# pyannote/pyannote-video

Measured on AMD Instinct MI355X. Metric: frames/sec end-to-end detect->embed->cluster, 1080p@25fps, higher is better.
Workload: dtype f32 (detector scores, embedder) / f64 (tracker, clustering) / u8 frames; an f16 screening pass with a proven error bound decides which windows the detector's exact f32 chain is evaluated for -- results identical to dense f32 scoring (`dense_scoring`)

## Files before the change

include/pvface.h:

```cpp
#ifndef PVFACE_H
#define PVFACE_H
#include <stdint.h>
#include <stddef.h>

#ifdef __cplusplus
extern "C" {
#endif

typedef uint64_t pvf_handle;
typedef struct { int32_t left, top, right, bottom; } pvf_rect_i32;

const char* pvf_last_error(void);
int32_t pvf_version(void);
int32_t pvf_device_count(int32_t* n);
int32_t pvf_ctx_create(int32_t device, pvf_handle* ctx);
int32_t pvf_ctx_create_prio(int32_t device, int32_t priority_class, pvf_handle* ctx);
int32_t pvf_ctx_destroy(pvf_handle ctx);
int32_t pvf_sync(pvf_handle ctx);

int32_t pvf_load_detector(pvf_handle ctx, const char* path);
int32_t pvf_load_shape_predictor(pvf_handle ctx, const char* path);
int32_t pvf_load_embedder(pvf_handle ctx, const char* path);
int32_t pvf_model_tensor(const char* path, int32_t kind, const char* name, void* out, int64_t cap_bytes, int64_t* nbytes);
int32_t pvf_set_tracker_tables(pvf_handle ctx, const double* mask64, const double* mask_scale, const double* tw64,
// ... 49 lines not shown
int32_t pvf_egress_create(pvf_handle ctx, int32_t out_w, int32_t out_h, int32_t depth, int32_t flags, pvf_handle* ring);
int32_t pvf_egress_destroy(pvf_handle ctx, pvf_handle ring);
int32_t pvf_egress_submit(pvf_handle ctx, pvf_handle ring, pvf_handle frame, const pvf_prim* prims, int32_t n_prims,
                          const uint8_t* text, int64_t text_bytes, int32_t* slot);
int32_t pvf_egress_wait(pvf_handle ctx, pvf_handle ring, int32_t slot, const uint8_t** host_planes);
int32_t pvf_egress_release(pvf_handle ctx, pvf_handle ring, int32_t slot);
int32_t pvf_debug_render_rgb(pvf_handle ctx, pvf_handle frame, int32_t out_w, int32_t out_h, const pvf_prim* prims, int32_t n_prims,
                             const uint8_t* text, int64_t text_bytes, uint8_t* rgb);
int32_t pvf_debug_redact_means(pvf_handle ctx, pvf_handle frame, int32_t out_w, int32_t out_h, const pvf_prim* prims, int32_t n_prims,
                               uint8_t* means, int64_t capacity);

int32_t pvf_detect(pvf_handle ctx, pvf_handle frame, int32_t upsample, double adjust_threshold,
                   pvf_rect_i32* out, float* scores, int32_t cap, int32_t* n);
int32_t pvf_detect_batch(pvf_handle ctx, const pvf_handle* frames, int32_t n_frames, int32_t upsample,
                         double adjust_threshold, pvf_rect_i32* out, float* scores, int32_t* counts,
                         int32_t cap_per_frame);
int32_t pvf_detect_many(pvf_handle ctx, const pvf_handle* frames, int32_t n_frames, int32_t batch, int32_t upsample,
                        double adjust_threshold, pvf_rect_i32* out, float* scores, int32_t* counts, int32_t cap);

int32_t pvf_detector_screening(pvf_handle ctx, int32_t on, int32_t list_cap);
int32_t pvf_detector_screening_stats(pvf_handle ctx, int64_t* batches, int64_t* listed, int64_t* retries, double* bounds, double* pipe_err);

int32_t pvf_embedder_split(pvf_handle ctx, int32_t on);
int32_t pvf_embedder_split_stats(pvf_handle ctx, int64_t* faces, int64_t* reruns, double* pipe_err);

int32_t pvf_tracker_create(pvf_handle ctx, pvf_handle* trk);
int32_t pvf_tracker_create_many(pvf_handle ctx, int32_t n, pvf_handle* trks);
int32_t pvf_tracker_destroy_many(pvf_handle ctx, const pvf_handle* trks, int32_t n);
int32_t pvf_tracker_clone_many(pvf_handle ctx, const pvf_handle* src, int32_t n, pvf_handle* dst);
int32_t pvf_tracker_destroy(pvf_handle ctx, pvf_handle trk);
int32_t pvf_tracker_start(pvf_handle ctx, pvf_handle trk, pvf_handle frame, const double box[4]);
int32_t pvf_tracker_update(pvf_handle ctx, pvf_handle trk, pvf_handle frame, double* psr);
int32_t pvf_tracker_position(pvf_handle ctx, pvf_handle trk, double box[4]);
int32_t pvf_tracker_start_many(pvf_handle ctx, const pvf_handle* trks, const pvf_handle* frames,
                               const double* boxes , int32_t n);
int32_t pvf_tracker_update_many(pvf_handle ctx, const pvf_handle* trks, const pvf_handle* frames, int32_t n,
                                double* psr , double* boxes_out );
int32_t pvf_tracker_update_many_deferred(pvf_handle ctx, const pvf_handle* trks, const pvf_handle* frames, int32_t n,
                                         double* psr, double* boxes_out);
int32_t pvf_tracker_commit_many(pvf_handle ctx, const pvf_handle* trks, const pvf_handle* frames, int32_t n);

int32_t pvf_overlap_matrix(const double* a, int32_t na, const double* b, int32_t nb, double ratio, double* out);
int32_t pvf_associate(const double* trackers, int32_t n_trackers, const double* detections, int32_t n_detections,
                      double min_overlap_ratio, int32_t* det_of_tracker);
int32_t pvf_munkres(const double* cost, int32_t n, int32_t* row_to_col);

// ... 219 lines not shown
```

pyannote-video_amd/csrc/api.hip:

```cpp
#include "pvf_internal.h"
#include <algorithm>
#include <cmath>
#include <cstdlib>
#include <string>
#include <thread>

#define API_BEGIN try {
#define API_END                                                        \
    return 0;                                                          \
    }                                                                  \
    catch (const std::exception& e) { pvf_set_error(e.what()); return -1; } \
    catch (...) { pvf_set_error("unknown error"); return -2; }

#define ENTER(c, h)                                                \
    Ctx* c = pvf_ctx(h);                                           \
    std::lock_guard<std::recursive_mutex> _api_lock(c->api_mu);    \
    HIP_CHECK(hipSetDevice(c->device))
#define ENTER_DET(c, h)                                            \
    Ctx* c = pvf_ctx(h);                                           \
    std::lock_guard<std::recursive_mutex> _det_lock(c->det_mu);    \
    HIP_CHECK(hipSetDevice(c->device))
#define ENTER_BOTH(c, h)                                           \
    Ctx* c = pvf_ctx(h);                                           \
    std::lock_guard<std::recursive_mutex> _det_lock(c->det_mu);    \
// ... 29 lines not shown
    PVF_REQUIRE(list_cap >= 0 && list_cap <= (1 << 26), "pvf_detector_screening: list_cap must be 0 (keep) .. 2^26");
    c->det_screen = on != 0;
    if (list_cap > 0) c->screen_list_cap = list_cap;
    API_END
}

extern "C" int32_t pvf_detector_screening_stats(pvf_handle h, int64_t* batches, int64_t* listed, int64_t* retries, double* bounds, double* pipe_err)
{
    API_BEGIN
    ENTER_DET(c, h);
    if (batches) *batches = c->screen_batches;
    if (listed) *listed = c->screen_listed;
    if (retries) *retries = c->screen_retries;
    if (bounds) for (int f = 0; f < c->det.n_filters; ++f) bounds[f] = c->det.screen_bound[f];
    if (pipe_err) *pipe_err = c->screen_pipe_err;
    API_END
}

extern "C" int32_t pvf_embedder_split(pvf_handle h, int32_t on)
{
    API_BEGIN
    ENTER(c, h);
    c->emb_split = on != 0;
    API_END
}

extern "C" int32_t pvf_embedder_split_stats(pvf_handle h, int64_t* faces, int64_t* reruns, double* pipe_err)
{
    API_BEGIN
    ENTER(c, h);
    if (faces) *faces = c->emb_split_faces;
    if (reruns) *reruns = c->emb_reruns;
    if (pipe_err) *pipe_err = c->emb_pipe_err;
    API_END
}

extern "C" int32_t pvf_detect_batch(pvf_handle h, const pvf_handle* frames, int32_t n_frames, int32_t upsample, double adjust,
                                    pvf_rect_i32* out, float* scores, int32_t* counts, int32_t cap)
{
    API_BEGIN
    ENTER_DET(c, h);
    PVF_REQUIRE(n_frames > 0 && frames && out && counts && cap > 0, "pvf_detect_batch: bad arguments");
    PVF_REQUIRE(upsample >= 0 && upsample <= 2, "pvf_detect_batch: upsample must be 0..2");
    std::vector<Frame> fr(n_frames);
    for (int i = 0; i < n_frames; ++i) fr[i] = c->frame(frames[i]);
    std::vector<std::vector<RawDet>> raw;
// ... 1160 lines not shown
```

pyannote-video_amd/csrc/ctx.hip:

```cpp
#include "pvf_internal.h"
#include "detect_ml.h"
#include <cmath>
#include <fstream>
#include <mutex>
#include <dlfcn.h>

static thread_local std::string g_err;
void pvf_set_error(const char* msg) { g_err = msg ? msg : ""; }
extern "C" const char* pvf_last_error(void) { return g_err.c_str(); }

static std::mutex g_ctx_mu;
static std::unordered_map<uint64_t, std::unique_ptr<Ctx>> g_ctxs;
static uint64_t g_next_ctx = 0x1000;

Ctx* pvf_ctx(pvf_handle h)
{
    std::lock_guard<std::mutex> lk(g_ctx_mu);
    auto it = g_ctxs.find(h);
    if (it == g_ctxs.end()) throw PvfError("unknown context handle");
    return it->second.get();
}

std::map<std::string, Tensor> pvf_read_container(const char* path)
{
// ... 264 lines not shown
{
    API_BEGIN
    int k = 0;
    if (hipGetDeviceCount(&k) != hipSuccess || k <= 0) throw PvfError("no HIP device visible: libpvface has no CPU fallback");
    PVF_REQUIRE(device >= 0 && device < k, "device index out of range");
    HIP_CHECK(hipSetDevice(device));
    hipDeviceProp_t prop;
    HIP_CHECK(hipGetDeviceProperties(&prop, device));
    if (strncmp(prop.gcnArchName, "gfx950", 6) != 0)
        throw PvfError(std::string("libpvface is built for gfx950 (MI355X) only; device is ") + prop.gcnArchName);
    std::unique_ptr<Ctx> c(new Ctx());
    c->device = device;
    c->n_cu = prop.multiProcessorCount;
    {
        int lo = 0, hi = 0;
        HIP_CHECK(hipDeviceGetStreamPriorityRange(&lo, &hi));
        int prio = priority_class < 0 ? lo : hi;
        if (const char* e = getenv("PVF_MAIN_STREAM_PRIO")) prio = (strcmp(e, "low") == 0) ? lo : hi;
        HIP_CHECK(hipStreamCreateWithPriority(&c->stream, hipStreamNonBlocking, priority_class == 2 ? lo : prio));
        HIP_CHECK(hipStreamCreateWithPriority(&c->det_stream, hipStreamNonBlocking, priority_class == 2 ? hi : lo));
    }
    if (const char* e = getenv("PVF_DETECTOR_SCREENING")) c->det_screen = atoi(e) != 0;
    if (const char* e = getenv("PVF_EMBEDDER_SPLIT")) c->emb_split = atoi(e) != 0;
    std::lock_guard<std::mutex> lk(g_ctx_mu);
    uint64_t id = g_next_ctx++;
    g_ctxs[id] = std::move(c);
    *out = id;
    API_END
}

extern "C" int32_t pvf_ctx_create(int32_t device, pvf_handle* out) { return pvf_ctx_create_prio(device, 0, out); }

extern "C" int32_t pvf_ctx_destroy(pvf_handle h)
{
    API_BEGIN
    Ctx* c = pvf_ctx(h);
    HIP_CHECK(hipSetDevice(c->device));
    (void)hipStreamSynchronize(c->stream);
    (void)hipStreamSynchronize(c->det_stream);
    for (auto& kv : c->frames) if (kv.second.owned) (void)hipFree((void*)kv.second.d);
    for (auto& kv : c->trackers) {
        Tracker& t = *kv.second;
        if (t.share) { if (--*t.share > 0) continue; delete t.share; t.share = nullptr; }
        if (t.d_state) (void)hipFree(t.d_state);
    }
    for (auto p : c->tracker_pool) (void)hipFree(p);
// ... 251 lines not shown
```

pyannote-video_amd/csrc/pvf_internal.h:

```cpp
#pragma once
#include <hip/hip_runtime.h>
#include <cstdint>
#include <cstdio>
#include <cstring>
#include <deque>
#include <map>
#include <atomic>
#include <memory>
#include <mutex>
#include <stdexcept>
#include <string>
#include <unordered_map>
#include <vector>
#include "../../include/pvface.h"
#include "scratch_layout.h"
#include "chip_plan.h"
#include "group_blocks.h"

#define PVF_FHOG_STRIDE 32

struct CandOverflow : PvfError { int needed; explicit CandOverflow(int n) : PvfError("detector: candidate buffer overflow"), needed(n) {} };
struct ScreenRetry : PvfError { ScreenRetry() : PvfError("detector: screening pass gave up") {} };

#define HIP_CHECK(expr)                                                                              \
// ... 186 lines not shown
    std::recursive_mutex api_mu;
    std::recursive_mutex det_mu;
    std::mutex frames_mu;
    std::mutex prof_mu;
    bool prof_on = false;
    std::map<std::string, ProfFamily> prof;
    std::vector<hipEvent_t> event_pool;
    DevBuf s_grad, s_pyr, s_hist, s_norm, s_feat, s_cand, s_misc, s_chip, s_chip_pyr, s_act0, s_act1, s_act2, s_trk0, s_trk1, s_trk2, s_trkfeat, s_clu0, s_clu1;
    HostBuf h_cand, h_misc;
    StageRing stage;
    DevBuf s_cand2[2], s_fptr[2];
    HostBuf h_cand2[2], h_fptr[2];
    hipEvent_t det_ev[2] = {nullptr, nullptr};
    int det_slot = 0;
    int det_cand_cap = 8192;
    bool det_screen = true, det_screen_suspended = false, screen_attr_set = false;
    int screen_list_cap = 1 << 20;
    DevBuf s_screen;
    int64_t screen_batches = 0, screen_listed = 0, screen_retries = 0;
    double screen_pipe_err = -1;
    bool screen_pipe_flushes_subnormals = false;
    bool emb_split = true, emb_probe_done = false;
    DevBuf s_emb_flags, s_emb_redo;
    DevBuf s_jit;
    bool jit_attr_set = false;
    int64_t emb_split_faces = 0, emb_reruns = 0;
    double emb_pipe_err = -1;
    int n_cu = 256;
    struct PoolBuf { uint8_t* p; hipEvent_t free_after; hipEvent_t free_after_det; };
    std::map<size_t, std::deque<PoolBuf>> frame_pool;
    size_t frame_pool_bytes = 0;
    void* ingest_rings = nullptr;
    void* render_state = nullptr;
    void* tube_state = nullptr;
    void* board_state = nullptr;
    struct MlPlanCache* ml_plans = nullptr;
    std::map<std::vector<int>, std::unique_ptr<DevBuf>> resize_tabs;
    const void* feat_ring_owner = nullptr;
    uint8_t* d_orient_lut = nullptr;
    uint8_t* d_wrap_lut = nullptr;
    DevBuf s_orb_set, s_orb_work;
    int orb_n = 0, orb_cap = 0;

    Frame frame(uint64_t id)
    {
        std::lock_guard<std::mutex> lk(frames_mu);
// ... 165 lines not shown
```

pyannote-video_amd/csrc/resnet.hip:

```cpp
#include "pvf_internal.h"
#include <cmath>
#include <cstdlib>
#include <cstring>
#include <vector>

typedef float f32x4 __attribute__((ext_vector_type(4)));
typedef uint32_t u32x4 __attribute__((ext_vector_type(4)));
typedef float f32x16 __attribute__((ext_vector_type(16)));
typedef _Float16 f16x8 __attribute__((ext_vector_type(8)));
typedef _Float16 f16x4 __attribute__((ext_vector_type(4)));
typedef uint32_t u32x2 __attribute__((ext_vector_type(2)));

void face_chip_details(const EmbedModel& m, const int32_t* pts, ChipDetails* out)
{
    const double size = m.chip_size, padding = m.chip_padding;
    double fx[51], fy[51], tx[51], ty[51];
    int n = 0;
    for (int i = 17; i < 68; ++i) {
        if ((55 <= i && i <= 59) || (65 <= i && i <= 67)) continue;
        if (17 <= i && i <= 26) continue;
        fx[n] = ((padding + (double)m.mean_shape[2 * (i - 17)]) / (2 * padding + 1)) * size;
        fy[n] = ((padding + (double)m.mean_shape[2 * (i - 17) + 1]) / (2 * padding + 1)) * size;
        tx[n] = pts[2 * i]; ty[n] = pts[2 * i + 1];
        ++n;
// ... 10 lines not shown
    }
    const double ca = a / s, cb = b / s;
    const double scale = std::sqrt(ca * ca + cb * cb);
    const double hx = size / 2.0, hy = size / 2.0;
    const double cx = (ca * (hx - mfx) - cb * (hy - mfy)) + mtx;
    const double cy = (cb * (hx - mfx) + ca * (hy - mfy)) + mty;
    const double wv = size * scale;
    out->l = cx - wv / 2; out->t = cy - wv / 2; out->r = cx + wv / 2; out->b = cy + wv / 2;
    out->cs = ca / scale; out->sn = cb / scale;
    out->rows = m.chip_size; out->cols = m.chip_size;
}

struct ConvArgs {
    const float* in; int B, H, W, Cin;
    const float* w; int K;
    const float* frag;
    const float* bias; const float* gamma; const float* beta;
    float* out; int OH, OW, Cout;
    int AH, AW;
    int ksz, stride, pad;
    int skip_mode;
    const float* skip; int XH, XW, XC, SH, SW;
    const uint32_t* wsplit; float out_scale; int* flags;
};


__device__ __forceinline__ int small_div(int x, int d, float rd)
{
    int q = (int)((float)x * rd);
    const int r = x - q * d;
    q += (r >= d) ? 1 : 0;
    q -= (r < 0) ? 1 : 0;
    return q;
}

template <int WM, int WN>
__device__ __forceinline__ void conv_epilogue(const ConvArgs& a, float* smem, const f32x16& acc0, const f32x16& acc1, long M, long m0, int n0,
                                              int rel0, int b_first, int hw, float r_hw, float r_ow, int wave, int lane)
{
    constexpr int PITCH = 36;
    const int wm = wave / WN, wn = wave % WN;
    const int li = lane & 31, kh = lane >> 5;
    const int col = n0 + wn * 32 + li;
    const float bias = a.bias[col], g = a.gamma[col], bt = a.beta[col];
    if (a.AH == a.OH && a.AW == a.OW && a.skip_mode != 2) {
        float* T = smem + wave * 64 * PITCH;
#pragma unroll
        for (int t = 0; t < 2; ++t)
#pragma unroll
            for (int reg = 0; reg < 16; ++reg)
                T[(t * 32 + (reg & 3) + 8 * (reg >> 2) + 4 * kh) * PITCH + li] = (t == 0 ? acc0[reg] : acc1[reg]);
        __builtin_amdgcn_wave_barrier();
        const int c4 = lane & 7, cb = n0 + wn * 32 + 4 * c4;
        const float4 bias4 = *reinterpret_cast<const float4*>(a.bias + cb), g4 = *reinterpret_cast<const float4*>(a.gamma + cb),
                     bt4 = *reinterpret_cast<const float4*>(a.beta + cb);
#pragma unroll
        for (int it = 0; it < 8; ++it) {
            const int row = it * 8 + (lane >> 3);
            const long m = m0 + wm * 64 + row;
            if (m >= M) continue;
            const float4 x = *reinterpret_cast<const float4*>(&T[row * PITCH + 4 * c4]);
            float4 v = make_float4((x.x + bias4.x) * g4.x + bt4.x, (x.y + bias4.y) * g4.y + bt4.y, (x.z + bias4.z) * g4.z + bt4.z,
                                   (x.w + bias4.w) * g4.w + bt4.w);
            if (a.skip_mode == 1) {
                const float4 sk = *reinterpret_cast<const float4*>(a.skip + (size_t)m * a.Cout + cb);
                v.x += sk.x; v.y += sk.y; v.z += sk.z; v.w += sk.w;
            }
            { v.x = v.x < 0.0f ? 0.0f : v.x; v.y = v.y < 0.0f ? 0.0f : v.y; v.z = v.z < 0.0f ? 0.0f : v.z; v.w = v.w < 0.0f ? 0.0f : v.w; }
            *reinterpret_cast<float4*>(a.out + (size_t)m * a.Cout + cb) = v;
        }
        return;
    }
#pragma unroll
    for (int t = 0; t < 2; ++t)
#pragma unroll
        for (int reg = 0; reg < 16; ++reg) {
            const int row = (reg & 3) + 8 * (reg >> 2) + 4 * kh;
            const long m = m0 + wm * 64 + t * 32 + row;
            if (m >= M) continue;
            const int rel = rel0 + wm * 64 + t * 32 + row;
            const int bb = small_div(rel, hw, r_hw);
            const int rem = rel - bb * hw;
            const int oy = small_div(rem, a.OW, r_ow);
            const int ox = rem - oy * a.OW;
            const int b = b_first + bb;
            float v = 0.0f;
            if (oy < a.AH && ox < a.AW) v = ((t == 0 ? acc0[reg] : acc1[reg]) + bias) * g + bt;
            if (a.skip_mode == 1) v += a.skip[(size_t)m * a.Cout + col];
            else if (a.skip_mode == 2) {
                if (col < a.XC && oy < a.SH && ox < a.SW) {
                    const float* q = a.skip + (((size_t)b * a.XH + 2 * oy) * a.XW + 2 * ox) * a.XC + col;
                    v += (((q[0] + q[a.XC]) + q[(size_t)a.XW * a.XC]) + q[(size_t)a.XW * a.XC + a.XC]) * 0.25f;
                }
            }
            if (v < 0.0f) v = 0.0f;
            a.out[(size_t)m * a.Cout + col] = v;
        }
}

struct ConvExact {
    static constexpr bool FLAGS = false;
    static constexpr int LANE_K = 16;
    static __device__ __forceinline__ const u32x4* weights(const ConvArgs& a) { return reinterpret_cast<const u32x4*>(a.w); }
    static __device__ __forceinline__ bool park_a(uint32_t* row, int j4, const u32x4& v)
    {
        *reinterpret_cast<uint2*>(row + 2 * j4) = make_uint2(v.x, v.z);
        *reinterpret_cast<uint2*>(row + 2 * j4 + 16) = make_uint2(v.y, v.w);
        return true;
    }
    static __device__ __forceinline__ void park_b(uint32_t* row, int j4, const u32x4& v) { park_a(row, j4, v); }
    static __device__ __forceinline__ void chunk(const uint32_t* pa0, const uint32_t* pa1, const uint32_t* pb, f32x16& acc0, f32x16& acc1)
    {
        f32x4 fa0[4], fa1[4], fb[4];
#pragma unroll
        for (int q = 0; q < 4; ++q) {
            fa0[q] = *reinterpret_cast<const f32x4*>(pa0 + 4 * q);
            fa1[q] = *reinterpret_cast<const f32x4*>(pa1 + 4 * q);
            fb[q] = *reinterpret_cast<const f32x4*>(pb + 4 * q);
        }
#pragma unroll
        for (int s = 0; s < 16; ++s) {
            acc0 = __builtin_amdgcn_mfma_f32_32x32x2f32(fa0[s >> 2][s & 3], fb[s >> 2][s & 3], acc0, 0, 0, 0);
            acc1 = __builtin_amdgcn_mfma_f32_32x32x2f32(fa1[s >> 2][s & 3], fb[s >> 2][s & 3], acc1, 0, 0, 0);
        }
    }
    static __device__ __forceinline__ void scale(const ConvArgs&, f32x16&, f32x16&) {}
};

#define EMB_A_SCALE_EXP 8
#define EMB_F16_LIMIT 65504.0f
struct ConvSplit {
    static constexpr bool FLAGS = true;
    static constexpr int LANE_K = 4;
    static __device__ __forceinline__ const u32x4* weights(const ConvArgs& a) { return reinterpret_cast<const u32x4*>(a.wsplit); }
    static __device__ __forceinline__ bool park_a(uint32_t* row, int j4, const u32x4& v)
    {
        const f32x4 xv = __builtin_bit_cast(f32x4, v) * (float)(1 << EMB_A_SCALE_EXP);
        const bool ok = __builtin_reduce_and(__builtin_elementwise_abs(xv) < EMB_F16_LIMIT);
        const f16x4 hi = __builtin_convertvector(xv, f16x4), lo = __builtin_convertvector(xv - __builtin_convertvector(hi, f32x4), f16x4);
        *reinterpret_cast<u32x2*>(row + 2 * j4) = __builtin_bit_cast(u32x2, hi);
        *reinterpret_cast<u32x2*>(row + 2 * j4 + 16) = __builtin_bit_cast(u32x2, lo);
        return ok;
    }
    static __device__ __forceinline__ void park_b(uint32_t* row, int j4, const u32x4& v) { *reinterpret_cast<u32x4*>(row + 4 * j4) = v; }
    static __device__ __forceinline__ void chunk(const uint32_t* pa0, const uint32_t* pa1, const uint32_t* pb, f32x16& acc0, f32x16& acc1)
    {
#pragma unroll
        for (int s = 0; s < 2; ++s) {
            const f16x8 ah0 = *reinterpret_cast<const f16x8*>(pa0 + 8 * s), al0 = *reinterpret_cast<const f16x8*>(pa0 + 16 + 8 * s);
            const f16x8 ah1 = *reinterpret_cast<const f16x8*>(pa1 + 8 * s), al1 = *reinterpret_cast<const f16x8*>(pa1 + 16 + 8 * s);
            const f16x8 bh = *reinterpret_cast<const f16x8*>(pb + 8 * s), bl = *reinterpret_cast<const f16x8*>(pb + 16 + 8 * s);
            acc0 = __builtin_amdgcn_mfma_f32_32x32x16_f16(ah0, bh, acc0, 0, 0, 0);
            acc1 = __builtin_amdgcn_mfma_f32_32x32x16_f16(ah1, bh, acc1, 0, 0, 0);
            acc0 = __builtin_amdgcn_mfma_f32_32x32x16_f16(ah0, bl, acc0, 0, 0, 0);
            acc1 = __builtin_amdgcn_mfma_f32_32x32x16_f16(ah1, bl, acc1, 0, 0, 0);
            acc0 = __builtin_amdgcn_mfma_f32_32x32x16_f16(al0, bh, acc0, 0, 0, 0);
            acc1 = __builtin_amdgcn_mfma_f32_32x32x16_f16(al1, bh, acc1, 0, 0, 0);
        }
    }
    static __device__ __forceinline__ void scale(const ConvArgs& a, f32x16& acc0, f32x16& acc1) { acc0 *= a.out_scale; acc1 *= a.out_scale; }
};

template <int WM, int WN, class Ops>
__global__ void __launch_bounds__(256) conv_tile_k(ConvArgs a)
{
    constexpr int BM = 64 * WM, BN = 32 * WN, KC = 32, PITCH = 36;
    static_assert(WM * WN == 4, "four waves per block");
    constexpr int SM_ROWS = (BM + BN > 256) ? BM + BN : 256;
    __shared__ __attribute__((aligned(16))) float smem[SM_ROWS * PITCH];
    uint32_t* As = reinterpret_cast<uint32_t*>(smem);
    uint32_t* Bs = As + BM * PITCH;
    const int tid = threadIdx.x, lane = tid & 63, wave = tid >> 6;
    const int wm = wave / WN, wn = wave % WN;
    const long M = (long)a.B * a.OH * a.OW;
    const long m0 = (long)blockIdx.x * BM;
    const int n0 = blockIdx.y * BN;
    f32x16 acc0, acc1;
#pragma unroll
    for (int i = 0; i < 16; ++i) { acc0[i] = 0.0f; acc1[i] = 0.0f; }

    constexpr int A_F4 = BM * 8 / 256, B_F4 = BN * 8 / 256;
    constexpr int RSRC_FLAGS = 0x00020000, OOB = (int)0x80000000;
    const int hw = a.OH * a.OW;
    const int b_first = (int)(m0 / hw);
    const int rel0 = (int)(m0 - (long)b_first * hw);
    const float r_hw = 1.0f / (float)hw, r_ow = 1.0f / (float)a.OW;
    const size_t face = (size_t)a.H * a.W * a.Cin;
    const size_t in_bytes = (size_t)(a.B - b_first) * face * sizeof(float);
    const __amdgpu_buffer_rsrc_t rs_in = __builtin_amdgcn_make_buffer_rsrc((void*)(a.in + (size_t)b_first * face), 0,
                                                                           in_bytes > 0x7ffffff0u ? 0x7ffffff0 : (int)in_bytes, RSRC_FLAGS);
    int pa_off[A_F4], pa_y[A_F4], pa_x[A_F4];
#pragma unroll
    for (int q = 0; q < A_F4; ++q) {
        const int i = (tid + q * 256) >> 3;
        const long m = m0 + i;
        pa_off[q] = 0; pa_y[q] = -(1 << 20); pa_x[q] = 0;
        if (m < M) {
            const int rel = rel0 + i;
            const int bb = small_div(rel, hw, r_hw);
            const int rem = rel - bb * hw;
            const int oy = small_div(rem, a.OW, r_ow);
            const int ox = rem - oy * a.OW;
            if (oy < a.AH && ox < a.AW) {
                pa_y[q] = oy * a.stride - a.pad; pa_x[q] = ox * a.stride - a.pad;
                pa_off[q] = ((bb * a.H + pa_y[q]) * a.W + pa_x[q]) * a.Cin;
            }
        }
    }
    const int Kpad = (a.K + KC - 1) / KC * KC;
    const int j4 = tid & 7;
    const u32x4* wrow[B_F4];
#pragma unroll
// ... 33 lines not shown
        for (int q = 0; q < B_F4; ++q) Ops::park_b(&Bs[((tid + q * 256) >> 3) * PITCH], j4, vb[q]);
        if constexpr (Ops::FLAGS)
            if (bad)
                for (int q = 0; q < A_F4; ++q)
                    if ((bad >> q) & 1) a.flags[b_first + small_div(rel0 + ((tid + q * 256) >> 3), hw, r_hw)] = 1;
    };
    const int li = lane & 31, kh = lane >> 5;
    const uint32_t* pa0 = &As[(wm * 64 + li) * PITCH + Ops::LANE_K * kh];
    const uint32_t* pa1 = pa0 + 32 * PITCH;
    const uint32_t* pb = &Bs[(wn * 32 + li) * PITCH + Ops::LANE_K * kh];
    offsets();
    issue();
    offsets();
    for (int k0 = 0; k0 < Kpad; k0 += KC) {
        park();
        __syncthreads();
        issue();
        __builtin_amdgcn_sched_barrier(0);
        offsets();
        Ops::chunk(pa0, pa1, pb, acc0, acc1);
        __syncthreads();
    }
    Ops::scale(a, acc0, acc1);
    conv_epilogue<WM, WN>(a, smem, acc0, acc1, M, m0, n0, rel0, b_first, hw, r_hw, r_ow, wave, lane);
}


__global__ void __launch_bounds__(256) conv_wsplit_k(const float* __restrict__ w, int total, int w_exp, _Float16* __restrict__ out)
{
    const int i = blockIdx.x * 256 + threadIdx.x;
    if (i >= total) return;
    const float v = ldexpf(w[i], w_exp);
    const _Float16 hi = (_Float16)v;
    const _Float16 lo = (_Float16)(v - (float)hi);
    const int row32 = i >> 5, kk = i & 31;
    out[(size_t)row32 * 64 + kk] = hi;
    out[(size_t)row32 * 64 + 32 + kk] = lo;
}

__global__ void __launch_bounds__(64) embed_probe_k(const uint4* __restrict__ a, const uint4* __restrict__ b, int steps, float* __restrict__ d)
{
    const int lane = threadIdx.x;
    f32x16 acc;
#pragma unroll
    for (int i = 0; i < 16; ++i) acc[i] = 0.0f;
    for (int s = 0; s < steps; ++s)
        acc = __builtin_amdgcn_mfma_f32_32x32x16_f16(__builtin_bit_cast(f16x8, a[s * 64 + lane]), __builtin_bit_cast(f16x8, b[s * 64 + lane]), acc, 0, 0, 0);
// ... 225 lines not shown
    float s = 0.0f;
    for (int i = 0; i < HW; ++i) s += x[((size_t)b * HW + i) * 256 + t];
    feat[t] = s / (float)HW;
    __syncthreads();
    if (t < 128) {
        float acc = 0.0f;
        for (int o = 0; o < 256; ++o) acc += feat[o] * fc[(size_t)o * 128 + t];
        out[(size_t)b * 128 + t] = acc;
    }
}

static bool conv_is_c32(const ConvArgs& a)
{
    return a.Cin == 32 && a.Cout == 32 && a.H == 35 && a.W == 35 && a.OH == 35 && a.OW == 35 && a.AH == 35 && a.AW == 35 && a.ksz == 3 &&
           a.stride == 1 && a.pad == 1 && a.skip_mode != 2;
}

static void launch_conv(Ctx* c, const ConvArgs& a)
{
    const long M = (long)a.B * a.OH * a.OW;
    PVF_REQUIRE(a.Cin % 32 == 0, "conv: input channels must be a multiple of 32 (the 3-channel first layer has a kernel of its own: stem_conv_k)");
    PVF_REQUIRE(a.OH * a.OW < (1 << 21) && a.Cout % 32 == 0, "conv: output map too large for the kernel's index arithmetic / Cout not a multiple of 32");
    auto tile = [&](auto exact, auto split, dim3 grid) { hipLaunchKernelGGL((a.wsplit ? split : exact), grid, dim3(256), 0, c->stream, a); };
    if (a.frag && conv_is_c32(a)) {
        static std::atomic<uint64_t> attr_set{0};
        const size_t lds = (size_t)(C32_TILE_FLOATS + 144 * 64) * sizeof(float);
        const uint64_t bit = 1ull << (c->device & 63);
        if (!(attr_set.load() & bit)) {
            HIP_CHECK(hipFuncSetAttribute(reinterpret_cast<const void*>(conv3x3_c32_k), hipFuncAttributeMaxDynamicSharedMemorySize, (int)lds));
            attr_set.fetch_or(bit);
        }
        const int items = a.B * (35 / C32_ROWS);
        hipLaunchKernelGGL(conv3x3_c32_k, dim3((unsigned)std::min(items, 2 * c->n_cu)), dim3(256), lds, c->stream, a.in, a.frag, a.bias, a.gamma, a.beta,
                           a.skip_mode == 1 ? a.skip : nullptr, a.out, items);
    } else if (a.Cout == 32) {
        tile(conv_tile_k<4, 1, ConvExact>, conv_tile_k<4, 1, ConvSplit>, dim3((unsigned)((M + 255) / 256), 1));
    } else {
        PVF_REQUIRE(a.Cout % 64 == 0, "conv: Cout must be 32 or a multiple of 64");
        tile(conv_tile_k<2, 2, ConvExact>, conv_tile_k<2, 2, ConvSplit>, dim3((unsigned)((M + 127) / 128), a.Cout / 64));
    }
}

void conv_layer_upload(ConvLayer& L, const float* w, const float* bias, const float* gamma, const float* beta)
{
    const int cin = L.cin, cout = L.cout, k = L.k;
    const int cp = (cin == 3) ? 4 : cin;
    const int K = k * k * cp, Kpad = (K + 31) / 32 * 32;
    std::vector<float> wt((size_t)cout * Kpad, 0.0f);
    for (int o = 0; o < cout; ++o)
        for (int ci = 0; ci < cin; ++ci)
            for (int r = 0; r < k; ++r)
                for (int s = 0; s < k; ++s) {
                    const int kk = (r * k + s) * cp + ci;
                    wt[(size_t)o * Kpad + kk] = w[(((size_t)o * cin + ci) * k + r) * k + s];
                }
    auto up = [](const float* src, size_t count) {
        float* d = nullptr;
        HIP_CHECK(hipMalloc((void**)&d, count * sizeof(float)));
        HIP_CHECK(hipMemcpy(d, src, count * sizeof(float), hipMemcpyHostToDevice));
        return d;
    };
    L.d_w = up(wt.data(), wt.size());
// ... 109 lines not shown

static const int UN[14][3] = {{32, 32, 0}, {32, 32, 0}, {32, 32, 0}, {32, 64, 1}, {64, 64, 0}, {64, 64, 0}, {64, 64, 0},
                              {64, 128, 1}, {128, 128, 0}, {128, 128, 0}, {128, 256, 1}, {256, 256, 0}, {256, 256, 0}, {256, 256, 1}};
struct UnitDims { int a, s, o; };
static UnitDims unit_dims(int u, int H)
{
    const int a = UN[u][2] ? 1 + (H - 3) / 2 : H, s = UN[u][2] ? 1 + (H - 2) / 2 : H;
    return {a, s, std::max(a, s)};
}

static void resnet_run(Ctx* c, const uint8_t* d_chips, int n, float* h_out, bool split, int* h_flags, const EmbedTap* tap = nullptr)
{
    const EmbedModel& e = c->emb;
    PVF_REQUIRE(e.loaded, "embedder not loaded");
    const int S = e.chip_size;
    const int MAXB = 4096;
    const int h1 = 1 + (S - 7) / 2;
    const int hp = 1 + (h1 - 3) / 2;
    const int cap = std::min(n, MAXB);
    const size_t big = (size_t)cap * h1 * h1 * 32;
    c->s_act0.ensure(std::max(big, (size_t)cap * S * S * 4) * sizeof(float));
    c->s_act1.ensure(big * sizeof(float));
    c->s_act2.ensure((size_t)cap * hp * hp * 32 * sizeof(float) + (size_t)cap * 128 * sizeof(float));
    PVF_REQUIRE(!tap || n <= MAXB, "embedder stage access: at most 4096 faces");
    auto tapped = [&](int stage, const float* d, int B, int H, int W, int C) {
        if (tap && tap->stage == stage && tap->h_out)
            HIP_CHECK(hipMemcpyAsync(tap->h_out, d, (size_t)B * H * W * C * sizeof(float), hipMemcpyDeviceToHost, c->stream));
    };
    for (int b0 = 0; b0 < n; b0 += MAXB) {
        const int B = std::min(MAXB, n - b0);
        ProfScope ps(c, "conv");
        float* x = c->s_act0.as<float>();
        float* y = c->s_act1.as<float>();
        float* z = c->s_act2.as<float>();
        const ConvLayer& L0 = e.convs[0];
        PVF_REQUIRE(S == 150 && L0.cout == 32 && L0.k == 7 && h1 == 72, "stem kernel: 150 x 150 chips, 7 x 7 stride 2, 32 channels");
        if (!c->emb.d_stem) {
            HIP_CHECK(hipMalloc(&c->emb.d_stem, STEM_NP * 64 * sizeof(float)));
            hipLaunchKernelGGL(stem_frag_k, dim3(STEM_NP), dim3(64), 0, c->stream, L0.d_w, c->emb.d_stem);
        }
        hipLaunchKernelGGL(stem_conv_k, dim3(h1 / STEM_ROWS, B), dim3(192), 0, c->stream, d_chips + (size_t)b0 * S * S * 3, B, c->emb.d_stem,
                           L0.d_bias, L0.d_gamma, L0.d_beta, y);
        tapped(0, y, B, h1, h1, 32);
        ConvArgs a;
        const size_t npool = (size_t)B * hp * hp * 32;
        hipLaunchKernelGGL(maxpool3s2_k, dim3((unsigned)((npool + 255) / 256)), dim3(256), 0, c->stream, y, B, h1, h1, 32, z, hp, hp);
        tapped(1, z, B, hp, hp, 32);
        float* cur = z; float* t1 = x; float* t2 = y;
        int H = hp;
        int* flags = nullptr;
        if (split) {
            flags = c->s_emb_flags.as<int>();
            HIP_CHECK(hipMemsetAsync(flags, 0, (size_t)B * sizeof(int), c->stream));
        }
        for (int u = 0; u < 14; ++u) {
            const int cin = UN[u][0], nn = UN[u][1], down = UN[u][2];
            ConvLayer& La = c->emb.convs[1 + 2 * u];
            ConvLayer& Lb = c->emb.convs[2 + 2 * u];
            const int stride = down ? 2 : 1, pad = down ? 0 : 1;
            const auto [ah, sh, oh] = unit_dims(u, H);
            memset(&a, 0, sizeof a);
            a.in = cur; a.B = B; a.H = H; a.W = H; a.Cin = cin;
            a.out = t1; a.OH = ah; a.OW = ah; a.Cout = nn; a.AH = ah; a.AW = ah; a.ksz = 3; a.stride = stride; a.pad = pad; a.skip_mode = 0;
            conv_bind_weights(c, La, split, false, flags, a);
            launch_conv(c, a);
            tapped(2 + 2 * u, t1, B, ah, ah, nn);
            memset(&a, 0, sizeof a);
            a.in = t1; a.B = B; a.H = ah; a.W = ah; a.Cin = nn;
            a.out = t2; a.OH = oh; a.OW = oh; a.Cout = nn; a.AH = ah; a.AW = ah; a.ksz = 3; a.stride = 1; a.pad = 1;
            a.skip_mode = down ? 2 : 1; a.skip = cur; a.XH = H; a.XW = H; a.XC = cin; a.SH = sh; a.SW = sh;
            conv_bind_weights(c, Lb, split, false, flags, a);
            launch_conv(c, a);
            tapped(3 + 2 * u, t2, B, oh, oh, nn);
            float* old = cur; cur = t2; t2 = old;
            H = oh;
        }
        float* d_out = reinterpret_cast<float*>(c->s_act2.as<uint8_t>() + (size_t)cap * hp * hp * 32 * sizeof(float));
        hipLaunchKernelGGL(head_k, dim3(B), dim3(256), 0, c->stream, cur, H * H, e.d_fc, d_out);
        HIP_CHECK(hipGetLastError());
        HIP_CHECK(hipMemcpyAsync(h_out + (size_t)b0 * 128, d_out, (size_t)B * 128 * sizeof(float), hipMemcpyDeviceToHost, c->stream));
        if (split) HIP_CHECK(hipMemcpyAsync(h_flags + b0, flags, (size_t)B * sizeof(int), hipMemcpyDeviceToHost, c->stream));
    }
    HIP_CHECK(hipStreamSynchronize(c->stream));
}

void resnet_forward(Ctx* c, const uint8_t* d_chips, int n, float* h_out)
{
    if (!c->emb_split) { resnet_run(c, d_chips, n, h_out, false, nullptr); return; }
    if (!c->emb_probe_done) { embed_probe(c); c->emb_probe_done = true; }
    c->s_emb_flags.ensure((size_t)std::min(n, 4096) * sizeof(int));
    std::vector<int> flags(n, 0);
    resnet_run(c, d_chips, n, h_out, true, flags.data());
    c->emb_split_faces += n;
    std::vector<int> redo;
    for (int i = 0; i < n; ++i) if (flags[i]) redo.push_back(i);
    if (redo.empty()) return;
    c->emb_reruns += (int64_t)redo.size();
// ... 108 lines not shown
```

pyannote-video_amd/pyannote_video_amd/_lib.py:

```python
import ctypes as C
import os
import numpy as np

_HERE = os.path.dirname(os.path.abspath(__file__))
LIB_PATH = os.environ.get("PVF_LIBRARY") or os.path.join(_HERE, "libpvface.so")

_lib = None


class PvfError(RuntimeError):
    pass


class OrbCapError(PvfError):

    def __init__(self, message, needed):
        PvfError.__init__(self, message)
        self.needed = int(needed)


class Rect(C.Structure):
    _fields_ = [("left", C.c_int32), ("top", C.c_int32), ("right", C.c_int32), ("bottom", C.c_int32)]


# ... 21 lines not shown
    "pvf_frame_device_ptr": (C.c_int32, [H, H, P]),
    "pvf_ingest_create": (C.c_int32, [H, C.c_int32, C.c_int32, C.c_int32, P]),
    "pvf_ingest_destroy": (C.c_int32, [H, H]),
    "pvf_ingest_acquire": (C.c_int32, [H, H, P, P]),
    "pvf_ingest_submit": (C.c_int32, [H, H, C.c_int32, P]),
    "pvf_ingest_wait": (C.c_int32, [H, H]),
    "pvf_ingest_create_yuv": (C.c_int32, [H, C.c_int32, C.c_int32, C.c_int32, C.c_int32, C.c_int32, P]),
    "pvf_frame_from_yuv": (C.c_int32, [H, P, C.c_int64, P, P, C.c_int64, C.c_int32, C.c_int32, C.c_int32, C.c_int32, C.c_int32, P]),
    "pvf_frame_resize": (C.c_int32, [H, H, C.c_int32, C.c_int32, P]),
    "pvf_render_batch": (C.c_int32, [H, P, C.c_int32, C.c_int32, C.c_int32, C.c_int32, P, P, P, C.c_int64, P, C.c_int32]),
    "pvf_egress_create": (C.c_int32, [H, C.c_int32, C.c_int32, C.c_int32, C.c_int32, P]),
    "pvf_egress_destroy": (C.c_int32, [H, H]),
    "pvf_egress_submit": (C.c_int32, [H, H, H, P, C.c_int32, P, C.c_int64, P]),
    "pvf_egress_wait": (C.c_int32, [H, H, C.c_int32, P]),
    "pvf_egress_release": (C.c_int32, [H, H, C.c_int32]),
    "pvf_debug_render_rgb": (C.c_int32, [H, H, C.c_int32, C.c_int32, P, C.c_int32, P, C.c_int64, P]),
    "pvf_debug_redact_means": (C.c_int32, [H, H, C.c_int32, C.c_int32, P, C.c_int32, P, C.c_int64]),
    "pvf_detect": (C.c_int32, [H, H, C.c_int32, C.c_double, P, P, C.c_int32, P]),
    "pvf_detect_batch": (C.c_int32, [H, P, C.c_int32, C.c_int32, C.c_double, P, P, P, C.c_int32]),
    "pvf_detect_many": (C.c_int32, [H, P, C.c_int32, C.c_int32, C.c_int32, C.c_double, P, P, P, C.c_int32]),
    "pvf_detector_screening": (C.c_int32, [H, C.c_int32, C.c_int32]),
    "pvf_detector_screening_stats": (C.c_int32, [H, P, P, P, P, P]),
    "pvf_embedder_split": (C.c_int32, [H, C.c_int32]),
    "pvf_embedder_split_stats": (C.c_int32, [H, P, P, P]),
    "pvf_tracker_create": (C.c_int32, [H, P]),
    "pvf_tracker_destroy": (C.c_int32, [H, H]),
    "pvf_tracker_create_many": (C.c_int32, [H, C.c_int32, P]),
    "pvf_tracker_destroy_many": (C.c_int32, [H, P, C.c_int32]),
    "pvf_tracker_clone_many": (C.c_int32, [H, P, C.c_int32, P]),
    "pvf_tracker_start": (C.c_int32, [H, H, H, P]),
    "pvf_tracker_update": (C.c_int32, [H, H, H, P]),
    "pvf_tracker_position": (C.c_int32, [H, H, P]),
    "pvf_tracker_start_many": (C.c_int32, [H, P, P, P, C.c_int32]),
    "pvf_tracker_update_many": (C.c_int32, [H, P, P, C.c_int32, P, P]),
    "pvf_tracker_update_many_deferred": (C.c_int32, [H, P, P, C.c_int32, P, P]),
    "pvf_tracker_commit_many": (C.c_int32, [H, P, P, C.c_int32]),
    "pvf_overlap_matrix": (C.c_int32, [P, C.c_int32, P, C.c_int32, C.c_double, P]),
    "pvf_munkres": (C.c_int32, [P, C.c_int32, P]),
    "pvf_associate": (C.c_int32, [P, C.c_int32, P, C.c_int32, C.c_double, P]),
    "pvf_landmarks": (C.c_int32, [H, P, P, C.c_int32, P]),
    "pvf_debug_landmarks_shape": (C.c_int32, [H, P, P, C.c_int32, P, P]),
    "pvf_embed": (C.c_int32, [H, P, P, C.c_int32, P]),
    "pvf_landmarks_embed": (C.c_int32, [H, P, P, C.c_int32, P, P]),
    "pvf_embed_chips": (C.c_int32, [H, P, C.c_int32, P]),
    "pvf_face_chips": (C.c_int32, [H, P, P, C.c_int32, P]),
    "pvf_chip_quality": (C.c_int32, [H, P, C.c_int32, P]),
# ... 226 lines not shown
```

pyannote-video_amd/pyannote_video_amd/runtime.py:

```python
import contextlib
import ctypes as C
import threading
import itertools
import operator
import numpy as np
from . import _lib
from ._lib import check, ptr, handles
from . import models as _models
from .y4m import YuvFrame, chroma_shape


class DeviceFrame(object):
    __slots__ = ("ctx", "handle", "height", "width", "keep", "transient", "__weakref__")

    def __init__(self, ctx, handle, height, width, keep=None, transient=False):
        self.ctx, self.handle, self.height, self.width, self.keep = ctx, handle, height, width, keep
        self.transient = transient

    @property
    def shape(self):
        return (self.height, self.width, 3)

    def release(self):
        if self.handle is not None and self.ctx._h is not None:
# ... 1249 lines not shown
                                                   ptr(e), C.byref(nb), int(flags)))
        else:
            check(self._l.pvf_cluster_dist(self._h, ptr(D), ptr(rs), T, float(threshold), ptr(labels), ptr(log), C.byref(n)))
        return labels, log[:n.value], nb.value

    def cluster_dist(self, D, row_start, threshold):
        return self._cluster_dist(D, row_start, threshold)[:2]

    def cluster_dist_cooccur(self, D, row_start, threshold, extent, flags=0):
        return self._cluster_dist(D, row_start, threshold, self._extent(extent, len(row_start) - 1), flags)

    def detector_screening(self, on=True, list_cap=0):
        check(self._l.pvf_detector_screening(self._h, 1 if on else 0, int(list_cap)))

    def detector_screening_stats(self):
        b, n, r, pe = C.c_int64(0), C.c_int64(0), C.c_int64(0), C.c_double(-1.0)
        bounds = np.zeros(8, np.float64)
        check(self._l.pvf_detector_screening_stats(self._h, C.byref(b), C.byref(n), C.byref(r), ptr(bounds), C.byref(pe)))
        return {"batches": b.value, "listed": n.value, "retries": r.value, "bounds": bounds[:5].tolist(), "pipe_err": pe.value}

    def embedder_split(self, on=True):
        check(self._l.pvf_embedder_split(self._h, 1 if on else 0))

    def embedder_split_stats(self):
        f, r, pe = C.c_int64(0), C.c_int64(0), C.c_double(-1.0)
        check(self._l.pvf_embedder_split_stats(self._h, C.byref(f), C.byref(r), C.byref(pe)))
        return {"faces": f.value, "reruns": r.value, "pipe_err": pe.value}

    def prof_enable(self, on=True):
        check(self._l.pvf_prof_enable(self._h, 1 if on else 0))

    def prof_reset(self):
        check(self._l.pvf_prof_reset(self._h))

    def prof_get(self, family):
        ms, n = C.c_double(0), C.c_int64(0)
        check(self._l.pvf_prof_get(self._h, family.encode(), C.byref(ms), C.byref(n)))
        return ms.value, n.value


def _seed64(seed):
    return int(seed) & 0xFFFFFFFFFFFFFFFF


_default = None

# ... 8 lines not shown
```

Before: 4717.

## Emit pre-split f16 hi/lo activation twins from conv epilogues for next layer

In the split (f16 hi/lo) embedder path, each 64-column conv now writes its ReLU output already split into scaled f16 hi/lo pairs. The following conv reads that twin directly instead of loading f32 activations and splitting them while staging A tiles, and the overflow flag check moves into the producer's epilogue. The aim is to remove the per-load conversion work and, for the first conv of each unit, skip the f32 output write. The cost is extra scratch memory for three twin buffers and extra twin writes for the second conv, whose f32 output is still needed for the skip path. The feature is on by default through a new toggle.

```diff
diff --git a/include/pvface.h b/include/pvface.h
--- a/include/pvface.h
+++ b/include/pvface.h
@@ -95,6 +95,7 @@
 int32_t pvf_detector_screening_stats(pvf_handle ctx, int64_t* batches, int64_t* listed, int64_t* retries, double* bounds, double* pipe_err);
 
 int32_t pvf_embedder_split(pvf_handle ctx, int32_t on);
+int32_t pvf_embedder_presplit(pvf_handle ctx, int32_t on);
 int32_t pvf_embedder_split_stats(pvf_handle ctx, int64_t* faces, int64_t* reruns, double* pipe_err);
 
 int32_t pvf_tracker_create(pvf_handle ctx, pvf_handle* trk);
diff --git a/pyannote-video_amd/csrc/api.hip b/pyannote-video_amd/csrc/api.hip
--- a/pyannote-video_amd/csrc/api.hip
+++ b/pyannote-video_amd/csrc/api.hip
@@ -75,6 +75,14 @@
     API_BEGIN
     ENTER(c, h);
     c->emb_split = on != 0;
+    API_END
+}
+
+extern "C" int32_t pvf_embedder_presplit(pvf_handle h, int32_t on)
+{
+    API_BEGIN
+    ENTER(c, h);
+    c->emb_presplit = on != 0;
     API_END
 }
 
diff --git a/pyannote-video_amd/csrc/ctx.hip b/pyannote-video_amd/csrc/ctx.hip
--- a/pyannote-video_amd/csrc/ctx.hip
+++ b/pyannote-video_amd/csrc/ctx.hip
@@ -310,6 +310,7 @@
     }
     if (const char* e = getenv("PVF_DETECTOR_SCREENING")) c->det_screen = atoi(e) != 0;
     if (const char* e = getenv("PVF_EMBEDDER_SPLIT")) c->emb_split = atoi(e) != 0;
+    if (const char* e = getenv("PVF_EMBEDDER_PRESPLIT")) c->emb_presplit = atoi(e) != 0;
     std::lock_guard<std::mutex> lk(g_ctx_mu);
     uint64_t id = g_next_ctx++;
     g_ctxs[id] = std::move(c);
diff --git a/pyannote-video_amd/csrc/pvf_internal.h b/pyannote-video_amd/csrc/pvf_internal.h
--- a/pyannote-video_amd/csrc/pvf_internal.h
+++ b/pyannote-video_amd/csrc/pvf_internal.h
@@ -232,6 +232,8 @@
     bool screen_pipe_flushes_subnormals = false;
     bool emb_split = true, emb_probe_done = false;
     DevBuf s_emb_flags, s_emb_redo;
+    bool emb_presplit = true;
+    DevBuf s_emb_twin;
     DevBuf s_jit;
     bool jit_attr_set = false;
     int64_t emb_split_faces = 0, emb_reruns = 0;
diff --git a/pyannote-video_amd/csrc/resnet.hip b/pyannote-video_amd/csrc/resnet.hip
--- a/pyannote-video_amd/csrc/resnet.hip
+++ b/pyannote-video_amd/csrc/resnet.hip
@@ -56,7 +56,21 @@
     int skip_mode;
     const float* skip; int XH, XW, XC, SH, SW;
     const uint32_t* wsplit; float out_scale; int* flags;
+    const uint32_t* in_twin; uint32_t* out_twin; int out_mode;
 };
+enum { CONV_OUT_F32 = 0, CONV_OUT_TWIN = 1, CONV_OUT_BOTH = 2 };
+
+#define EMB_A_SCALE_EXP 8
+#define EMB_F16_LIMIT 65504.0f
+__device__ __forceinline__ bool split_quad(const f32x4& v, u32x2& hi2, u32x2& lo2)
+{
+    const f32x4 xv = v * (float)(1 << EMB_A_SCALE_EXP);
+    const bool ok = __builtin_reduce_and(__builtin_elementwise_abs(xv) < EMB_F16_LIMIT);
+    const f16x4 hi = __builtin_convertvector(xv, f16x4), lo = __builtin_convertvector(xv - __builtin_convertvector(hi, f32x4), f16x4);
+    hi2 = __builtin_bit_cast(u32x2, hi);
+    lo2 = __builtin_bit_cast(u32x2, lo);
+    return ok;
+}
 
 
 __device__ __forceinline__ int small_div(int x, int d, float rd)
@@ -68,7 +82,7 @@
     return q;
 }
 
-template <int WM, int WN>
+template <int WM, int WN, bool TWIN>
 __device__ __forceinline__ void conv_epilogue(const ConvArgs& a, float* smem, const f32x16& acc0, const f32x16& acc1, long M, long m0, int n0,
                                               int rel0, int b_first, int hw, float r_hw, float r_ow, int wave, int lane)
 {
@@ -101,7 +115,16 @@
                 v.x += sk.x; v.y += sk.y; v.z += sk.z; v.w += sk.w;
             }
             { v.x = v.x < 0.0f ? 0.0f : v.x; v.y = v.y < 0.0f ? 0.0f : v.y; v.z = v.z < 0.0f ? 0.0f : v.z; v.w = v.w < 0.0f ? 0.0f : v.w; }
-            *reinterpret_cast<float4*>(a.out + (size_t)m * a.Cout + cb) = v;
+            if (!TWIN || a.out_mode != CONV_OUT_TWIN) *reinterpret_cast<float4*>(a.out + (size_t)m * a.Cout + cb) = v;
+            if constexpr (TWIN)
+                if (a.out_mode != CONV_OUT_F32) {
+                    u32x2 hi, lo;
+                    const bool ok = split_quad(f32x4{v.x, v.y, v.z, v.w}, hi, lo);
+                    uint32_t* tw = a.out_twin + (size_t)m * a.Cout + (n0 + wn * 32) + 2 * c4;
+                    *reinterpret_cast<u32x2*>(tw) = hi;
+                    *reinterpret_cast<u32x2*>(tw + 16) = lo;
+                    if (!ok) a.flags[b_first + small_div(rel0 + wm * 64 + row, hw, r_hw)] = 1;
+                }
         }
         return;
     }
@@ -128,13 +151,23 @@
                 }
             }
             if (v < 0.0f) v = 0.0f;
-            a.out[(size_t)m * a.Cout + col] = v;
+            if (!TWIN || a.out_mode != CONV_OUT_TWIN) a.out[(size_t)m * a.Cout + col] = v;
+            if constexpr (TWIN)
+                if (a.out_mode != CONV_OUT_F32) {
+                    const float xv = v * (float)(1 << EMB_A_SCALE_EXP);
+                    const _Float16 hi = (_Float16)xv, lo = (_Float16)(xv - (float)hi);
+                    _Float16* tw = reinterpret_cast<_Float16*>(a.out_twin + (size_t)m * a.Cout + (n0 + wn * 32)) + li;
+                    tw[0] = hi;
+                    tw[32] = lo;
+                    if (!(fabsf(xv) < EMB_F16_LIMIT)) a.flags[b] = 1;
+                }
         }
 }
 
 struct ConvExact {
-    static constexpr bool FLAGS = false;
+    static constexpr bool FLAGS = false, TWIN_OUT = false;
     static constexpr int LANE_K = 16;
+    static __device__ __forceinline__ const void* input(const ConvArgs& a) { return a.in; }
     static __device__ __forceinline__ const u32x4* weights(const ConvArgs& a) { return reinterpret_cast<const u32x4*>(a.w); }
     static __device__ __forceinline__ bool park_a(uint32_t* row, int j4, const u32x4& v)
     {
@@ -161,19 +194,17 @@
     static __device__ __forceinline__ void scale(const ConvArgs&, f32x16&, f32x16&) {}
 };
 
-#define EMB_A_SCALE_EXP 8
-#define EMB_F16_LIMIT 65504.0f
 struct ConvSplit {
-    static constexpr bool FLAGS = true;
+    static constexpr bool FLAGS = true, TWIN_OUT = false;
     static constexpr int LANE_K = 4;
+    static __device__ __forceinline__ const void* input(const ConvArgs& a) { return a.in; }
     static __device__ __forceinline__ const u32x4* weights(const ConvArgs& a) { return reinterpret_cast<const u32x4*>(a.wsplit); }
     static __device__ __forceinline__ bool park_a(uint32_t* row, int j4, const u32x4& v)
     {
-        const f32x4 xv = __builtin_bit_cast(f32x4, v) * (float)(1 << EMB_A_SCALE_EXP);
-        const bool ok = __builtin_reduce_and(__builtin_elementwise_abs(xv) < EMB_F16_LIMIT);
-        const f16x4 hi = __builtin_convertvector(xv, f16x4), lo = __builtin_convertvector(xv - __builtin_convertvector(hi, f32x4), f16x4);
-        *reinterpret_cast<u32x2*>(row + 2 * j4) = __builtin_bit_cast(u32x2, hi);
-        *reinterpret_cast<u32x2*>(row + 2 * j4 + 16) = __builtin_bit_cast(u32x2, lo);
+        u32x2 hi, lo;
+        const bool ok = split_quad(__builtin_bit_cast(f32x4, v), hi, lo);
+        *reinterpret_cast<u32x2*>(row + 2 * j4) = hi;
+        *reinterpret_cast<u32x2*>(row + 2 * j4 + 16) = lo;
         return ok;
     }
     static __device__ __forceinline__ void park_b(uint32_t* row, int j4, const u32x4& v) { *reinterpret_cast<u32x4*>(row + 4 * j4) = v; }
@@ -193,6 +224,12 @@
         }
     }
     static __device__ __forceinline__ void scale(const ConvArgs& a, f32x16& acc0, f32x16& acc1) { acc0 *= a.out_scale; acc1 *= a.out_scale; }
+};
+struct ConvSplitTwin : ConvSplit { static constexpr bool TWIN_OUT = true; };
+struct ConvPresplit : ConvSplit {
+    static constexpr bool FLAGS = false, TWIN_OUT = true;
+    static __device__ __forceinline__ const void* input(const ConvArgs& a) { return a.in_twin; }
+    static __device__ __forceinline__ bool park_a(uint32_t* row, int j4, const u32x4& v) { park_b(row, j4, v); return true; }
 };
 
 template <int WM, int WN, class Ops>
@@ -221,7 +258,7 @@
     const float r_hw = 1.0f / (float)hw, r_ow = 1.0f / (float)a.OW;
     const size_t face = (size_t)a.H * a.W * a.Cin;
     const size_t in_bytes = (size_t)(a.B - b_first) * face * sizeof(float);
-    const __amdgpu_buffer_rsrc_t rs_in = __builtin_amdgcn_make_buffer_rsrc((void*)(a.in + (size_t)b_first * face), 0,
+    const __amdgpu_buffer_rsrc_t rs_in = __builtin_amdgcn_make_buffer_rsrc((void*)(static_cast<const float*>(Ops::input(a)) + (size_t)b_first * face), 0,
                                                                            in_bytes > 0x7ffffff0u ? 0x7ffffff0 : (int)in_bytes, RSRC_FLAGS);
     int pa_off[A_F4], pa_y[A_F4], pa_x[A_F4];
 #pragma unroll
@@ -301,7 +338,7 @@
         __syncthreads();
     }
     Ops::scale(a, acc0, acc1);
-    conv_epilogue<WM, WN>(a, smem, acc0, acc1, M, m0, n0, rel0, b_first, hw, r_hw, r_ow, wave, lane);
+    conv_epilogue<WM, WN, Ops::TWIN_OUT>(a, smem, acc0, acc1, M, m0, n0, rel0, b_first, hw, r_hw, r_ow, wave, lane);
 }
 
 
@@ -573,6 +610,10 @@
     PVF_REQUIRE(a.Cin % 32 == 0, "conv: input channels must be a multiple of 32 (the 3-channel first layer has a kernel of its own: stem_conv_k)");
     PVF_REQUIRE(a.OH * a.OW < (1 << 21) && a.Cout % 32 == 0, "conv: output map too large for the kernel's index arithmetic / Cout not a multiple of 32");
     auto tile = [&](auto exact, auto split, dim3 grid) { hipLaunchKernelGGL((a.wsplit ? split : exact), grid, dim3(256), 0, c->stream, a); };
+    const bool twin_in = a.in_twin != nullptr, twin_out = a.out_mode != CONV_OUT_F32;
+    PVF_REQUIRE(!twin_out || (a.out_twin && a.flags), "conv: a split twin is asked for without its buffer or the faces' flags");
+    PVF_REQUIRE((!twin_in && !twin_out) || (a.wsplit && a.Cout % 64 == 0 && !(a.frag && conv_is_c32(a))),
+                "conv: split twins belong to the split form of the 64-column tile");
     if (a.frag && conv_is_c32(a)) {
         static std::atomic<uint64_t> attr_set{0};
         const size_t lds = (size_t)(C32_TILE_FLOATS + 144 * 64) * sizeof(float);
@@ -588,7 +629,10 @@
         tile(conv_tile_k<4, 1, ConvExact>, conv_tile_k<4, 1, ConvSplit>, dim3((unsigned)((M + 255) / 256), 1));
     } else {
         PVF_REQUIRE(a.Cout % 64 == 0, "conv: Cout must be 32 or a multiple of 64");
-        tile(conv_tile_k<2, 2, ConvExact>, conv_tile_k<2, 2, ConvSplit>, dim3((unsigned)((M + 127) / 128), a.Cout / 64));
+        const dim3 grid((unsigned)((M + 127) / 128), a.Cout / 64);
+        if (twin_in) hipLaunchKernelGGL((conv_tile_k<2, 2, ConvPresplit>), grid, dim3(256), 0, c->stream, a);
+        else if (twin_out) hipLaunchKernelGGL((conv_tile_k<2, 2, ConvSplitTwin>), grid, dim3(256), 0, c->stream, a);
+        else tile(conv_tile_k<2, 2, ConvExact>, conv_tile_k<2, 2, ConvSplit>, grid);
     }
 }
 
@@ -744,6 +788,14 @@
     c->s_act0.ensure(std::max(big, (size_t)cap * S * S * 4) * sizeof(float));
     c->s_act1.ensure(big * sizeof(float));
     c->s_act2.ensure((size_t)cap * hp * hp * 32 * sizeof(float) + (size_t)cap * 128 * sizeof(float));
+    const bool presplit = split && c->emb_presplit;
+    ScratchLayout twin_lay;
+    ScratchSlot<uint32_t> twin_slot[3];
+    if (presplit) {
+        const int h64 = unit_dims(3, hp).o;
+        for (auto& s : twin_slot) s = twin_lay.take<uint32_t>((size_t)cap * h64 * h64 * 64);
+        c->s_emb_twin.ensure(twin_lay.bytes());
+    }
     PVF_REQUIRE(!tap || n <= MAXB, "embedder stage access: at most 4096 faces");
     auto tapped = [&](int stage, const float* d, int B, int H, int W, int C) {
         if (tap && tap->stage == stage && tap->h_out)
@@ -775,16 +827,23 @@
             flags = c->s_emb_flags.as<int>();
             HIP_CHECK(hipMemsetAsync(flags, 0, (size_t)B * sizeof(int), c->stream));
         }
+        uint32_t *cur_tw = nullptr, *t1_tw = nullptr, *t2_tw = nullptr, *spare_tw = nullptr;
+        if (presplit) { t1_tw = twin_slot[0].in(c->s_emb_twin); t2_tw = twin_slot[1].in(c->s_emb_twin); spare_tw = twin_slot[2].in(c->s_emb_twin); }
         for (int u = 0; u < 14; ++u) {
             const int cin = UN[u][0], nn = UN[u][1], down = UN[u][2];
             ConvLayer& La = c->emb.convs[1 + 2 * u];
             ConvLayer& Lb = c->emb.convs[2 + 2 * u];
             const int stride = down ? 2 : 1, pad = down ? 0 : 1;
             const auto [ah, sh, oh] = unit_dims(u, H);
+            const bool twins = presplit && !(cin == 32 && nn == 32);
+            const bool tap_a = tap && tap->stage == 2 + 2 * u && tap->h_out;
             memset(&a, 0, sizeof a);
             a.in = cur; a.B = B; a.H = H; a.W = H; a.Cin = cin;
             a.out = t1; a.OH = ah; a.OW = ah; a.Cout = nn; a.AH = ah; a.AW = ah; a.ksz = 3; a.stride = stride; a.pad = pad; a.skip_mode = 0;
             conv_bind_weights(c, La, split, false, flags, a);
+            if (twins) {
+                a.in_twin = cur_tw; a.out_twin = t1_tw; a.out_mode = tap_a ? CONV_OUT_BOTH : CONV_OUT_TWIN;
+            }
             launch_conv(c, a);
             tapped(2 + 2 * u, t1, B, ah, ah, nn);
             memset(&a, 0, sizeof a);
@@ -792,9 +851,14 @@
             a.out = t2; a.OH = oh; a.OW = oh; a.Cout = nn; a.AH = ah; a.AW = ah; a.ksz = 3; a.stride = 1; a.pad = 1;
             a.skip_mode = down ? 2 : 1; a.skip = cur; a.XH = H; a.XW = H; a.XC = cin; a.SH = sh; a.SW = sh;
             conv_bind_weights(c, Lb, split, false, flags, a);
+            if (twins) {
+                a.in_twin = t1_tw;
+                if (u < 13) { a.out_twin = t2_tw; a.out_mode = CONV_OUT_BOTH; }
+            }
             launch_conv(c, a);
             tapped(3 + 2 * u, t2, B, oh, oh, nn);
             float* old = cur; cur = t2; t2 = old;
+            if (twins) { uint32_t* o = cur_tw ? cur_tw : spare_tw; cur_tw = t2_tw; t2_tw = o; }
             H = oh;
         }
         float* d_out = reinterpret_cast<float*>(c->s_act2.as<uint8_t>() + (size_t)cap * hp * hp * 32 * sizeof(float));
diff --git a/pyannote-video_amd/pyannote_video_amd/_lib.py b/pyannote-video_amd/pyannote_video_amd/_lib.py
--- a/pyannote-video_amd/pyannote_video_amd/_lib.py
+++ b/pyannote-video_amd/pyannote_video_amd/_lib.py
@@ -67,6 +67,7 @@
     "pvf_detector_screening": (C.c_int32, [H, C.c_int32, C.c_int32]),
     "pvf_detector_screening_stats": (C.c_int32, [H, P, P, P, P, P]),
     "pvf_embedder_split": (C.c_int32, [H, C.c_int32]),
+    "pvf_embedder_presplit": (C.c_int32, [H, C.c_int32]),
     "pvf_embedder_split_stats": (C.c_int32, [H, P, P, P]),
     "pvf_tracker_create": (C.c_int32, [H, P]),
     "pvf_tracker_destroy": (C.c_int32, [H, H]),
diff --git a/pyannote-video_amd/pyannote_video_amd/runtime.py b/pyannote-video_amd/pyannote_video_amd/runtime.py
--- a/pyannote-video_amd/pyannote_video_amd/runtime.py
+++ b/pyannote-video_amd/pyannote_video_amd/runtime.py
@@ -1295,6 +1295,9 @@
     def embedder_split(self, on=True):
         check(self._l.pvf_embedder_split(self._h, 1 if on else 0))
 
+    def embedder_presplit(self, on=True):
+        check(self._l.pvf_embedder_presplit(self._h, 1 if on else 0))
+
     def embedder_split_stats(self):
         f, r, pe = C.c_int64(0), C.c_int64(0), C.c_double(-1.0)
         check(self._l.pvf_embedder_split_stats(self._h, C.byref(f), C.byref(r), C.byref(pe)))
```

Result: faster. 4815, median of 5 (+2.1%).
